# Huangtianyu-caas/MAGOT

Hardware: NVIDIA B200
Metric: spliced+translated Gbp/s (higher is better)
Workload: dtype u8

## Files before the change

magot_b200/csrc/mg_common.cuh:

```cuda
#pragma once
#include <cuda_runtime.h>
#include <stdint.h>
#include <stdio.h>
#include <atomic>
#include <string>
#include <vector>
#include "../../include/magot_b200.h"

#define MG_FRONT_PAD 64
#define MG_TAIL_WORDS 8
#define MG_CODE_EXC 15u

void mg_set_error(const char *fmt, ...);
extern std::atomic<int64_t> g_mg_launches;
#define MG_COUNT_LAUNCH() (++g_mg_launches)

#define MG_CUDA(call)                                                                             \
    do {                                                                                          \
        cudaError_t _e = (call);                                                                  \
        if (_e != cudaSuccess) {                                                                  \
            mg_set_error("%s failed at %s:%d: %s", #call, __FILE__, __LINE__, cudaGetErrorString(_e)); \
            return MG_ECUDA;                                                                      \
        }                                                                                         \
    } while (0)
// ... 35 lines not shown
    bool finalized = false;
    uint64_t generation = 0;
    uint8_t *d_stage = nullptr;
    int64_t stage_cap = 0;
    uint8_t *d_raw = nullptr;
    unsigned long long *d_strip_tmp = nullptr;
    int64_t raw_cap = 0;
    uint8_t *h_pin = nullptr;
    int64_t pin_cap = 0;
    uint8_t *d_aa4096 = nullptr;
    uint8_t *d_aa4096h = nullptr;
    uint32_t *d_stops = nullptr;
    int64_t stop_words = 0;
    bool stops_valid = false;
    uint32_t *d_stops_alt = nullptr;
    uint64_t stops_alt_key = 0;
    bool stops_alt_valid = false;
    mg_sixframe_state *six = nullptr;
    int64_t device_bytes = 0;
};

struct mg_plan {
    mg_genome *g = nullptr;
    int device = 0;
    int64_t n_rec = 0, n_seg = 0, n_piece = 0, n_lit = 0;
    int64_t *d_rec_seg_off = nullptr;
    int32_t *d_seg_contig = nullptr;
    int64_t *d_seg_start = nullptr, *d_seg_end = nullptr;
    int8_t *d_seg_strand = nullptr;
    int64_t *d_rec_lit_off = nullptr;
    int32_t *d_rec_pre = nullptr, *d_rec_suf = nullptr;
    int8_t *d_rec_phase = nullptr;
    uint8_t *d_lit = nullptr;
    int64_t *d_blk_r0 = nullptr;
    int64_t *d_piece_src = nullptr;
    int64_t *d_piece_off = nullptr;
    int64_t *d_prot_off = nullptr;
    int32_t *d_rec_aa = nullptr;
    int8_t *d_rec_skip = nullptr;
    int64_t *d_nuc_tile = nullptr;
    int64_t *d_prot_tile = nullptr;
    int64_t n_nuc_tile = 0, n_prot_tile = 0;
    int32_t *d_blk1k = nullptr;
    int64_t blk1k_cap = 0;
    bool blk1k_ready = false;
    int64_t max_seg_per_rec = 0;
    int64_t nuc_upper = 0;
    int64_t *d_tile_buf = nullptr;
    int64_t tile_cap = 0;
    cudaStream_t last_stream = 0;
    int64_t *d_scan_tmp = nullptr;
    int64_t scan_tmp_cap = 0;
    int64_t nuc_total = -1, prot_total = -1;
    int64_t *d_totals = nullptr;
    bool totals_known = false;
    int prot_flags = 0;
    bool prepared = false;
    uint64_t generation = 0;
    bool prot_ready = false;
    unsigned long long *rec_tmp = nullptr;
    int64_t rec_tmp_words = 0;
    int64_t *rec_tile = nullptr;
    uint32_t *d_order = nullptr;
    int64_t order_cap = 0;
    uint8_t *d_out = nullptr;
    int64_t out_cap = 0;
    uint8_t *d_aa8192 = nullptr;
    bool own_code = false;
    std::vector<void *> owned;
};

#define MG_KIND_FWD 0ull
#define MG_KIND_RC 1ull
#define MG_KIND_LIT 2ull
#define MG_KIND_SHIFT 62
#define MG_SRC_MASK ((1ull << MG_KIND_SHIFT) - 1ull)

#ifndef MG_NUC_TILE
#define MG_NUC_TILE 32768
#endif
#ifndef MG_PROT_TILE
#define MG_PROT_TILE 16384
#endif

void build_aa4096(uint8_t *t, const uint8_t *codon64);
int mg_plan_check_prepared(const mg_plan *p);
// ... 115 lines not shown
```

magot_b200/csrc/mg_plan.cu:

```cuda
#include <algorithm>
#include <cstdlib>
#include <cstring>
#include "mg_common.cuh"
#include "mg_gather.cuh"
#include "mg_lookback.cuh"


#define PLAN_ITEMS 4
#define PLAN_TILE (256 * PLAN_ITEMS)

__global__ void __launch_bounds__(256) k_plan_block_rec(int64_t n_block, int64_t n_rec, const int64_t *__restrict__ rec_seg_off,
                                                        int64_t *__restrict__ blk_r0) {
    const int64_t r = blockIdx.x * (int64_t)blockDim.x + threadIdx.x;
    if (r >= n_rec) return;
    const int64_t f0 = __ldg(rec_seg_off + r) + 2 * r, f1 = __ldg(rec_seg_off + r + 1) + 2 * (r + 1);
    for (int64_t b = (f0 + PLAN_TILE - 1) / PLAN_TILE; b * PLAN_TILE < f1 && b < n_block; b++) blk_r0[b] = r;
}

#ifndef PLAN_MINB
#define PLAN_MINB 8
#endif
__global__ void __launch_bounds__(256, PLAN_MINB) k_plan_pieces(int64_t n_piece, int64_t n_rec, const int64_t *__restrict__ rec_seg_off,
                                                     const int64_t *__restrict__ blk_r0,
                                                     const int32_t *__restrict__ seg_contig, const int64_t *__restrict__ seg_start,
                                                     const int64_t *__restrict__ seg_end, const int8_t *__restrict__ seg_strand,
                                                     const int64_t *__restrict__ rec_lit_off, const int32_t *__restrict__ rec_pre,
                                                     const int32_t *__restrict__ rec_suf, const int64_t *__restrict__ contig_len,
                                                     const int64_t *__restrict__ contig_base, int64_t n_contigs, int64_t two_T,
                                                     unsigned long long *tmp, int64_t *__restrict__ piece_off,
                                                     int64_t *__restrict__ piece_src, int64_t *__restrict__ total_out,
                                                     int64_t *__restrict__ tile_first, int64_t tile_cap,
                                                     int32_t *__restrict__ blk1k, int64_t blk1k_cap) {
    __shared__ int64_t s_F[PLAN_TILE / 2 + 2];
    __shared__ int64_t s_warp[8];
    __shared__ int64_t s_prefix;
    __shared__ unsigned int s_tile;
    const int64_t tile = mg_next_tile(tmp, &s_tile);
    const int64_t pb = tile * PLAN_TILE;
    const int64_t r0 = blk_r0[tile];
    for (int i = threadIdx.x; i < PLAN_TILE / 2 + 2; i += blockDim.x) {
        const int64_t r = r0 + i;
        s_F[i] = r <= n_rec ? __ldg(rec_seg_off + r) + 2 * r : INT64_MAX;
    }
    __syncthreads();
    int64_t len[PLAN_ITEMS];
    const int64_t p0 = pb + (int64_t)threadIdx.x * PLAN_ITEMS;
    int lo = 0;
#pragma unroll
    for (int it = 0; it < PLAN_ITEMS; it++) {
        const int64_t p = p0 + it;
        len[it] = 0;
        if (p < n_piece) {
            if (it == 0) {
                int hi = PLAN_TILE / 2 + 1;
                while (hi - lo > 1) {
                    const int mid = (lo + hi) >> 1;
                    if (s_F[mid] <= p) lo = mid; else hi = mid;
                }
            } else {
                while (s_F[lo + 1] <= p) lo++;
            }
            const int64_t r = r0 + lo;
            const int64_t s0 = s_F[lo] - 2 * r, s1 = s_F[lo + 1] - 2 * (r + 1);
            const int64_t local = p - (s0 + 2 * r);
            if (local == 0) {
                len[it] = rec_pre[r];
                piece_src[p] = rec_lit_off[r] | (int64_t)(MG_KIND_LIT << MG_KIND_SHIFT);
            } else if (local == s1 - s0 + 1) {
                len[it] = rec_suf[r];
                piece_src[p] = (rec_lit_off[r] + rec_pre[r]) | (int64_t)(MG_KIND_LIT << MG_KIND_SHIFT);
            } else {
                const int64_t e = s0 + local - 1;
                const int32_t c = seg_contig[e];
                int64_t src = MG_FRONT_PAD, n = 0;
                if (c >= 0 && c < n_contigs) {
                    const int64_t L = contig_len[c];
                    int64_t i = seg_start[e] - 1, j = seg_end[e];
                    if (i < 0) { i += L; if (i < 0) i = 0; } else if (i > L) i = L;
                    if (j < 0) { j += L; if (j < 0) j = 0; } else if (j > L) j = L;
                    n = j > i ? j - i : 0;
                    if (n > 0x7fffffff) n = 0x7fffffff;
                    src = contig_base[c] + i;
                }
                len[it] = n;
                piece_src[p] = seg_strand[e] ? two_T - src - n : src;
            }
        }
    }
    int64_t mine = 0;
#pragma unroll
    for (int it = 0; it < PLAN_ITEMS; it++) mine += len[it];
    int64_t total;
    const int64_t incl = mg_block_incl_scan(mine, s_warp, &total);
    const int64_t prefix = mg_lookback(tmp, tile, total, &s_prefix);
    int64_t run = prefix + incl - mine;
#pragma unroll
    for (int it = 0; it < PLAN_ITEMS; it++) {
        if (p0 + it < n_piece) {
            piece_off[p0 + it] = run;
            if (tile_first && len[it] > 0) {
                for (int64_t t = (run + MG_NUC_TILE - 1) / MG_NUC_TILE; t * MG_NUC_TILE < run + len[it] && t < tile_cap; t++)
                    tile_first[t] = p0 + it;
            }
            if (blk1k_cap > 0 && len[it] > 0) {
                for (int64_t t = (run + 1023) >> 10; (t << 10) < run + len[it] && t < blk1k_cap; t++) blk1k[t] = (int32_t)(p0 + it);
            }
        }
        run += len[it];
    }
    if (tile == gridDim.x - 1 && threadIdx.x == 0) {
        const int64_t all = prefix + total;
        piece_off[n_piece] = all;
        *total_out = all;
        if (tile_first) {
            const int64_t n_tile = min(tile_cap, (all + MG_NUC_TILE - 1) / MG_NUC_TILE);
            tile_first[n_tile] = n_piece > 0 ? n_piece - 1 : 0;
        }
        const int64_t n_blk = (all + 1023) >> 10;
        if (n_blk < blk1k_cap) blk1k[n_blk] = (int32_t)(n_piece > 0 ? n_piece - 1 : 0);
    }
}

__global__ void __launch_bounds__(256) k_plan_records(int64_t n_rec, const int64_t *__restrict__ rec_seg_off,
                                                      const int64_t *__restrict__ piece_off, const int64_t *__restrict__ piece_src,
                                                      const uint32_t *__restrict__ packed, const int8_t *__restrict__ rec_phase,
                                                      int flags, int32_t *__restrict__ rec_aa, int8_t *__restrict__ rec_skip,
                                                      unsigned long long *tmp, int64_t *__restrict__ prot_off,
                                                      int64_t *__restrict__ total_out, int64_t *__restrict__ tile_first,
                                                      int64_t tile_cap) {
    __shared__ int64_t s_warp[8];
    __shared__ int64_t s_prefix;
    __shared__ unsigned int s_tile;
    const int64_t tile = mg_next_tile(tmp, &s_tile);
    const int64_t r = tile * (int64_t)blockDim.x + threadIdx.x;
    int64_t plen = 0;
    if (r < n_rec) {
    const int64_t f0 = rec_seg_off[r] + 2 * r, f1 = rec_seg_off[r + 1] + 2 * (r + 1);
    const int64_t pay0 = piece_off[f0 + 1], pay1 = piece_off[f1 - 1];
    const int64_t pre = pay0 - piece_off[f0], suf = piece_off[f1] - pay1;
    int64_t L = pay1 - pay0;
    int skip = 0;
    if ((flags & MG_PROT_USE_PHASE) && rec_phase) { skip = rec_phase[r]; if (skip < 0 || skip > 2) skip = 0; }
    L -= skip;
    int64_t naa;
    if (L <= 2) {
        naa = -1;
    } else {
        naa = L / 3;
        if (flags & MG_PROT_TRIMX) {
            uint64_t acc[3];
            const int64_t S = pay0 + skip;
            int64_t j = f0 + 1;
            while (j + 1 < f1 - 1 && __ldg(piece_off + j + 1) <= S) j++;
            mg_gather_nib(packed, piece_off, piece_src, j, S, 3, acc);
            const uint32_t n3 = (uint32_t)acc[0] & 0xFFFu;
            if (n3 & 0x888u) { naa -= 1; skip += 3; }
        }
    }
    if (naa > 0x7fffffff) naa = 0x7fffffff;
    rec_aa[r] = (int32_t)naa;
    rec_skip[r] = (int8_t)skip;
    plen = pre + (naa > 0 ? naa : 0) + suf;
    }
    int64_t total;
    const int64_t incl = mg_block_incl_scan(plen, s_warp, &total);
    const int64_t prefix = mg_lookback(tmp, tile, total, &s_prefix);
    if (r < n_rec) {
        const int64_t off = prefix + incl - plen;
        prot_off[r] = off;
        if (tile_first && plen > 0) {
            for (int64_t t = (off + MG_PROT_TILE - 1) / MG_PROT_TILE; t * MG_PROT_TILE < off + plen && t < tile_cap; t++) tile_first[t] = r;
        }
    }
    if (tile == gridDim.x - 1 && threadIdx.x == blockDim.x - 1) {
        const int64_t all = prefix + total;
        prot_off[n_rec] = all;
        *total_out = all;
        if (tile_first) {
            const int64_t n_tile = min(tile_cap, (all + MG_PROT_TILE - 1) / MG_PROT_TILE);
            tile_first[n_tile] = n_rec > 0 ? n_rec - 1 : 0;
        }
    }
}


#define PR_THREADS 256
#ifndef PR_MAXSEG
#define PR_MAXSEG 256
#endif

struct pr_seg { int64_t src; int64_t n; };

__device__ __forceinline__ pr_seg pr_clamp(int64_t e, const int32_t *__restrict__ seg_contig, const int64_t *__restrict__ seg_start,
                                           const int64_t *__restrict__ seg_end, const int8_t *__restrict__ seg_strand,
                                           const int64_t *__restrict__ contig_len, const int64_t *__restrict__ contig_base,
                                           int64_t n_contigs, int64_t two_T) {
    const int32_t c = __ldg(seg_contig + e);
    int64_t src = MG_FRONT_PAD, n = 0;
    if (c >= 0 && c < n_contigs) {
        const int64_t L = __ldg(contig_len + c);
        int64_t i = __ldg(seg_start + e) - 1, j = __ldg(seg_end + e);
        if (i < 0) { i += L; if (i < 0) i = 0; } else if (i > L) i = L;
        if (j < 0) { j += L; if (j < 0) j = 0; } else if (j > L) j = L;
        n = j > i ? j - i : 0;
        if (n > 0x7fffffff) n = 0x7fffffff;
        src = __ldg(contig_base + c) + i;
    }
// ... 192 lines not shown
    MG_REQUIRE(n_seg == 0 || (seg_contig && seg_start && seg_end && seg_strand), "segment arrays are NULL");
    MG_REQUIRE(n_rec == 0 || (rec_lit_off && rec_pre_len && rec_suf_len), "record arrays are NULL");
    MG_REQUIRE(rec_seg_off[0] == 0 && rec_seg_off[n_rec] == n_seg, "rec_seg_off must start at 0 and end at n_seg");
    MG_REQUIRE(n_seg + 2 * n_rec < 0x7fffffff, "more than 2^31 pieces in one plan: split the table");
    MG_CUDA(cudaSetDevice(g->device));
    cudaStream_t st = (cudaStream_t)stream;
    mg_plan *p = new mg_plan();
    p->g = g;
    p->device = g->device;
    p->n_rec = n_rec;
    p->n_seg = n_seg;
    p->n_piece = n_seg + 2 * n_rec;
    p->n_lit = n_lit;
    p->last_stream = st;
    int rc = MG_OK;
#define TRY(x) do { rc = (x); if (rc) { mg_plan_destroy(p); return rc; } } while (0)
    TRY(upload(p, &p->d_rec_seg_off, rec_seg_off, n_rec + 1, st));
    TRY(upload(p, &p->d_seg_contig, seg_contig, n_seg, st));
    TRY(upload(p, &p->d_seg_start, seg_start, n_seg, st));
    TRY(upload(p, &p->d_seg_end, seg_end, n_seg, st));
    TRY(upload(p, &p->d_seg_strand, seg_strand, n_seg, st));
    TRY(upload(p, &p->d_rec_lit_off, rec_lit_off, n_rec, st));
    TRY(upload(p, &p->d_rec_pre, rec_pre_len, n_rec, st));
    TRY(upload(p, &p->d_rec_suf, rec_suf_len, n_rec, st));
    {
        uint8_t *d = nullptr;
        TRY(dalloc(p, &d, n_lit + 128, st));
        rc = cudaMemsetAsync(d, 0, n_lit + 128, st) == cudaSuccess ? MG_OK : MG_ECUDA;
        if (rc == MG_OK && n_lit > 0 && cudaMemcpyAsync(d + 64, lit, n_lit, cudaMemcpyHostToDevice, st) != cudaSuccess) rc = MG_ECUDA;
        if (rc) { mg_set_error("literal upload failed"); mg_plan_destroy(p); return rc; }
        p->d_lit = d + 64;
    }
    if (rec_phase) TRY(upload(p, &p->d_rec_phase, rec_phase, n_rec, st));
    TRY(dalloc(p, &p->d_blk_r0, (p->n_piece + PLAN_TILE - 1) / PLAN_TILE + 1, st));
    {
        int64_t up = 0;
        for (int64_t e = 0; e < n_seg; e++) {
            int64_t d = seg_end[e] - seg_start[e] + 1;
            const int32_t c = seg_contig[e];
            const int64_t L = (c >= 0 && c < g->n_contigs) ? g->h_contig_len[c] : 0;
            if (seg_start[e] > seg_end[e] || d > L) d = L;
            if (d > 0) up += d < 0x7fffffff ? d : 0x7fffffff;
        }
        for (int64_t r = 0; r < n_rec; r++) up += (int64_t)rec_pre_len[r] + rec_suf_len[r];
        p->nuc_upper = up;
        p->blk1k_cap = (up >> 10) + 3;
        TRY(dalloc(p, &p->d_blk1k, p->blk1k_cap, st));
    }
    TRY(dalloc(p, &p->d_piece_src, p->n_piece, st));
    TRY(dalloc(p, &p->d_piece_off, p->n_piece + 1, st));
    TRY(dalloc(p, &p->d_prot_off, n_rec + 1, st));
    TRY(dalloc(p, &p->d_rec_aa, n_rec, st));
    TRY(dalloc(p, &p->d_rec_skip, n_rec, st));
    p->scan_tmp_cap = (p->n_piece + PLAN_TILE - 1) / PLAN_TILE + 1 + 2 * ((n_rec + 127) / 128 + 1) + 2;
    for (int64_t r = 0; r < n_rec; r++) p->max_seg_per_rec = std::max(p->max_seg_per_rec, rec_seg_off[r + 1] - rec_seg_off[r]);
    TRY(dalloc(p, &p->d_scan_tmp, p->scan_tmp_cap, st));
#undef TRY
    if (n_rec > 0) {
        const int64_t n_block = (p->n_piece + PLAN_TILE - 1) / PLAN_TILE, n_rblock = (n_rec + 255) / 256;
        k_plan_block_rec<<<(unsigned)n_rblock, 256, 0, st>>>(n_block, n_rec, p->d_rec_seg_off, p->d_blk_r0);
        MG_COUNT_LAUNCH();
        if (cudaGetLastError() != cudaSuccess) { mg_set_error("k_plan_block_rec launch failed"); mg_plan_destroy(p); return MG_ECUDA; }
    }
    *out = p;
    return MG_OK;
}

extern "C" int mg_plan_destroy(mg_plan *p) {
    if (!p) return MG_OK;
    cudaSetDevice(p->device);
    for (void *d : p->owned) cudaFreeAsync(d, p->last_stream);
    if (p->d_out) cudaFreeAsync(p->d_out, p->last_stream);
    delete p;
    return MG_OK;
}

extern "C" int mg_plan_set_codon_table(mg_plan *p, const uint8_t *codon64) {
    MG_REQUIRE(p != nullptr, "plan handle is NULL");
    if (!codon64) { p->own_code = false; return MG_OK; }
    for (int c = 0; c < 64; c++) MG_REQUIRE(codon64[c] != 'X', "codon64 maps an A/C/G/T codon to 'X'");
    MG_CUDA(cudaSetDevice(p->device));
    uint8_t t[8192];
    build_aa4096(t, codon64);
    for (uint32_t c = 0; c < 4096; c++) t[4096 + mg_aa_slot(c)] = t[c];
    cudaStream_t st = p->last_stream;
    if (!p->d_aa8192) {
        int rc = dalloc(p, &p->d_aa8192, 8192, st);
        if (rc) return rc;
    }
    MG_CUDA(cudaMemcpyAsync(p->d_aa8192, t, 8192, cudaMemcpyHostToDevice, st));
    MG_CUDA(cudaStreamSynchronize(st));
    p->own_code = true;
    return MG_OK;
}

static int plan_alloc_tiles(mg_plan *p, int64_t cap_nuc, int64_t cap_prot, cudaStream_t st);
static int64_t plan_tile_need(int64_t cap_nuc, int64_t cap_prot) {
    return (cap_nuc + MG_NUC_TILE - 1) / MG_NUC_TILE + 1 + (cap_prot + MG_PROT_TILE - 1) / MG_PROT_TILE + 1;
}
static int64_t pr_tiles(const mg_plan *p) { return (p->n_rec + PR_RECS - 1) / PR_RECS; }

static int plan_launch_records(mg_plan *p, cudaStream_t st);
static int plan_launch_scans(mg_plan *p, int prot_flags, cudaStream_t st, bool scatter_tiles = false, int64_t cap_nuc = 0,
                             int64_t cap_prot = 0) {
    mg_genome *g = p->g;
    p->prot_flags = prot_flags;
    p->last_stream = st;
    p->prot_ready = false;
    const int64_t n_block = (p->n_piece + PLAN_TILE - 1) / PLAN_TILE, n_rblock = (p->n_rec + 255) / 256;
    unsigned long long *tmp_a = reinterpret_cast<unsigned long long *>(p->d_scan_tmp), *tmp_b = tmp_a + n_block + 1;
    p->d_totals = reinterpret_cast<int64_t *>(tmp_b + n_rblock + 1);
    const bool one_launch = p->n_rec > 0 && p->max_seg_per_rec <= PR_MAXSEG && mg_k1_mode() == 1;
    if (p->n_rec == 0) MG_CUDA(cudaMemsetAsync(p->d_scan_tmp, 0, p->scan_tmp_cap * sizeof(int64_t), st));
    else if (one_launch) MG_CUDA(cudaMemsetAsync(p->d_scan_tmp, 0, 2 * (pr_tiles(p) + 1) * sizeof(unsigned long long), st));
    else MG_CUDA(cudaMemsetAsync(tmp_a, 0, (n_block + 1) * sizeof(unsigned long long), st));
    int64_t *tf_nuc = nullptr, *tf_prot = nullptr;
    if (scatter_tiles) {
        int rc = plan_alloc_tiles(p, cap_nuc, cap_prot, st);
        if (rc) return rc;
        tf_nuc = p->d_nuc_tile;
        tf_prot = p->d_prot_tile;
    }
    if (p->n_rec == 0) { p->prot_ready = true; return MG_OK; }
    if (one_launch) {
        const int64_t n_tile = pr_tiles(p);
        unsigned long long *ta = reinterpret_cast<unsigned long long *>(p->d_scan_tmp), *tb = ta + n_tile + 1;
        p->d_totals = reinterpret_cast<int64_t *>(p->d_scan_tmp + p->scan_tmp_cap - 2);
        k_plan_rec<<<(unsigned)n_tile, PR_THREADS, 0, st>>>(
            p->n_rec, p->n_piece, p->d_rec_seg_off, p->d_seg_contig, p->d_seg_start, p->d_seg_end, p->d_seg_strand, p->d_rec_lit_off,
            p->d_rec_pre, p->d_rec_suf, p->d_rec_phase, prot_flags, g->d_contig_len, g->d_contig_base, g->n_contigs, 2 * g->total_bases,
            g->d_packed, ta, tb, p->d_piece_off, p->d_piece_src, p->d_prot_off, p->d_rec_aa, p->d_rec_skip, p->d_totals, tf_nuc,
            p->n_nuc_tile, tf_prot, p->n_prot_tile, p->d_blk1k, p->blk1k_cap);
        MG_LAUNCH_CHECK();
        p->prot_ready = true;
        p->blk1k_ready = true;
        return MG_OK;
    }
    const bool want_blk1k = mg_emit_mode() == 2;
    p->blk1k_ready = want_blk1k;
    k_plan_pieces<<<(unsigned)n_block, 256, 0, st>>>(
        p->n_piece, p->n_rec, p->d_rec_seg_off, p->d_blk_r0, p->d_seg_contig, p->d_seg_start, p->d_seg_end, p->d_seg_strand,
        p->d_rec_lit_off, p->d_rec_pre, p->d_rec_suf, g->d_contig_len, g->d_contig_base, g->n_contigs, 2 * g->total_bases,
        tmp_a, p->d_piece_off, p->d_piece_src, p->d_totals, tf_nuc, p->n_nuc_tile, p->d_blk1k, want_blk1k ? p->blk1k_cap : 0);
    MG_LAUNCH_CHECK();
    p->rec_tmp = tmp_b;
    p->rec_tmp_words = n_rblock + 1;
    p->rec_tile = tf_prot;
    if (prot_flags & MG_PROT_DEFER) return MG_OK;
    return plan_launch_records(p, st);
}

static int plan_launch_records(mg_plan *p, cudaStream_t st) {
    mg_genome *g = p->g;
    const int64_t n_rblock = (p->n_rec + 255) / 256;
    MG_CUDA(cudaMemsetAsync(p->rec_tmp, 0, p->rec_tmp_words * sizeof(unsigned long long), st));
    k_plan_records<<<(unsigned)n_rblock, 256, 0, st>>>(
        p->n_rec, p->d_rec_seg_off, p->d_piece_off, p->d_piece_src, g->d_packed, p->d_rec_phase, p->prot_flags,
        p->d_rec_aa, p->d_rec_skip, p->rec_tmp, p->d_prot_off, p->d_totals + 1, p->rec_tile, p->n_prot_tile);
    MG_LAUNCH_CHECK();
    p->prot_ready = true;
    return MG_OK;
}

int mg_plan_check_prepared(const mg_plan *p) {
    if (!p->prepared) { mg_set_error("mg_plan_prepare has not been called"); return MG_ESTATE; }
    if (p->generation != p->g->generation) {
        mg_set_error("the genome changed (pack, finalize or mask) since the plan was prepared: prepare it again");
        return MG_ESTATE;
    }
    return MG_OK;
}

extern "C" int mg_plan_prepare_prot_async(mg_plan *p, void *stream) {
    MG_REQUIRE(p != nullptr, "plan handle is NULL");
    if (!p->prepared) { mg_set_error("mg_plan_prepare_async has not been called"); return MG_ESTATE; }
    if (const int rc0 = mg_plan_check_prepared(p)) return rc0;
    if (p->prot_ready || p->n_rec == 0) return MG_OK;
    MG_CUDA(cudaSetDevice(p->device));
    p->last_stream = (cudaStream_t)stream;
    return plan_launch_records(p, (cudaStream_t)stream);
}

static int plan_alloc_tiles(mg_plan *p, int64_t cap_nuc, int64_t cap_prot, cudaStream_t st) {
    p->n_nuc_tile = (cap_nuc + MG_NUC_TILE - 1) / MG_NUC_TILE;
    p->n_prot_tile = (cap_prot + MG_PROT_TILE - 1) / MG_PROT_TILE;
    const int64_t tile_need = plan_tile_need(cap_nuc, cap_prot);
    if (tile_need > p->tile_cap) {
        void *d = nullptr;
        MG_CUDA(cudaMallocAsync(&d, tile_need * sizeof(int64_t), st));
        p->owned.push_back(d);
        p->d_tile_buf = (int64_t *)d;
        p->tile_cap = tile_need;
    }
    p->d_nuc_tile = p->d_tile_buf;
    p->d_prot_tile = p->d_tile_buf + p->n_nuc_tile + 1;
    return MG_OK;
}

static int plan_launch_tiles(mg_plan *p, int64_t cap_nuc, int64_t cap_prot, cudaStream_t st) {
    int rc = plan_alloc_tiles(p, cap_nuc, cap_prot, st);
    if (rc) return rc;
    if (p->n_rec > 0 && p->n_nuc_tile + p->n_prot_tile > 0) {
        k_plan_tiles<<<(unsigned)((p->n_nuc_tile + p->n_prot_tile + 2 + 255) / 256), 256, 0, st>>>(
            p->d_totals, p->d_piece_off, p->n_piece, MG_NUC_TILE, p->n_nuc_tile, p->d_nuc_tile, p->d_prot_off, p->n_rec, MG_PROT_TILE,
            p->n_prot_tile, p->d_prot_tile);
        MG_LAUNCH_CHECK();
    }
    return MG_OK;
}

static int plan_read_totals(mg_plan *p, cudaStream_t st, int64_t totals[2]) {
    totals[0] = totals[1] = 0;
// ... 9 lines not shown
    MG_CUDA(cudaSetDevice(p->device));
    cudaStream_t st = (cudaStream_t)stream;
    p->prepared = false;
    int rc = plan_launch_scans(p, prot_flags & ~MG_PROT_DEFER, st);
    if (rc) return rc;
    int64_t totals[2];
    rc = plan_read_totals(p, st, totals);
    if (rc) return rc;
    p->nuc_total = totals[0];
    p->prot_total = totals[1];
    p->totals_known = true;
    rc = plan_launch_tiles(p, p->nuc_total, p->prot_total, st);
    if (rc) return rc;
    p->prepared = true;
    p->generation = p->g->generation;
    if (nuc_total) *nuc_total = p->nuc_total;
    if (prot_total) *prot_total = p->prot_total;
    return MG_OK;
}

extern "C" int mg_plan_prepare_async(mg_plan *p, int prot_flags, int64_t nuc_capacity, int64_t prot_capacity, void *stream) {
    MG_REQUIRE(p != nullptr, "plan handle is NULL");
    MG_REQUIRE(nuc_capacity >= 0 && prot_capacity >= 0, "capacities must be >= 0");
    MG_CUDA(cudaSetDevice(p->device));
    if (plan_tile_need(nuc_capacity, prot_capacity) > p->tile_cap) {
        const int rc0 = mg_refuse_growth_in_capture((cudaStream_t)stream, "mg_plan_prepare_async (first prepare, or larger capacities)");
        if (rc0) return rc0;
    }
    p->prepared = false;
    int rc = plan_launch_scans(p, prot_flags, (cudaStream_t)stream, true, nuc_capacity, prot_capacity);
    if (rc) return rc;
    p->nuc_total = nuc_capacity;
    p->prot_total = prot_capacity;
    p->totals_known = false;
    p->prepared = true;
    p->generation = p->g->generation;
    return MG_OK;
}

extern "C" int mg_plan_totals(mg_plan *p, int64_t *nuc_total, int64_t *prot_total, void *stream) {
    MG_REQUIRE(p != nullptr, "plan handle is NULL");
    if (const int rc0 = mg_plan_check_prepared(p)) return rc0;
    MG_CUDA(cudaSetDevice(p->device));
    if (!p->totals_known) {
        int64_t totals[2];
        int rc = plan_read_totals(p, (cudaStream_t)stream, totals);
        if (rc) return rc;
        if (!p->prot_ready) totals[1] = 0;
        if (totals[0] > p->nuc_total || totals[1] > p->prot_total) {
            mg_set_error("text sizes (%lld nucleotide, %lld protein bytes) exceed the capacities given to mg_plan_prepare_async "
                         "(%lld, %lld): the emitted texts are truncated", (long long)totals[0], (long long)totals[1],
                         (long long)p->nuc_total, (long long)p->prot_total);
            return MG_EINVAL;
        }
        p->nuc_total = totals[0];
        p->prot_total = totals[1];
        p->totals_known = true;
    }
    if (nuc_total) *nuc_total = p->nuc_total;
    if (prot_total) *prot_total = p->prot_total;
    return MG_OK;
}

extern "C" int mg_plan_lengths(mg_plan *p, int64_t *nuc_len, int64_t *aa_len, void *stream) {
    MG_REQUIRE(p != nullptr, "plan handle is NULL");
    if (const int rc0 = mg_plan_check_prepared(p)) return rc0;
// ... 16 lines not shown
```

Measured before the change: 1938.

## Precompute per-piece descriptors to replace binary search in plan pieces kernel

Replaces the per-tile record index and the shared-memory binary search in k_plan_pieces with a precomputed int32 descriptor per piece: either a segment index, or an encoded record prefix/suffix literal. The pieces kernel then reads the descriptors with vector loads and issues segment and literal loads in batches to raise memory-level parallelism, keeping lengths in shared memory. Tile-first and blk1k writes are skipped when a thread's range does not cross a tile boundary. The record kernel gains a fast path that reads the first codon directly when it lies within the first piece. In exchange it adds an n_piece-sized descriptor buffer and limits indices to 32 bits.

Result: faster. 1976, median of 6 (+2.0%).

```diff
diff --git a/magot_b200/csrc/mg_common.cuh b/magot_b200/csrc/mg_common.cuh
--- a/magot_b200/csrc/mg_common.cuh
+++ b/magot_b200/csrc/mg_common.cuh
@@ -91,7 +91,7 @@
     int32_t *d_rec_pre = nullptr, *d_rec_suf = nullptr;
     int8_t *d_rec_phase = nullptr;
     uint8_t *d_lit = nullptr;
-    int64_t *d_blk_r0 = nullptr;
+    int32_t *d_piece_desc = nullptr;
     int64_t *d_piece_src = nullptr;
     int64_t *d_piece_off = nullptr;
     int64_t *d_prot_off = nullptr;
diff --git a/magot_b200/csrc/mg_plan.cu b/magot_b200/csrc/mg_plan.cu
--- a/magot_b200/csrc/mg_plan.cu
+++ b/magot_b200/csrc/mg_plan.cu
@@ -6,22 +6,28 @@
 #include "mg_lookback.cuh"
 
 
+#ifndef PLAN_ITEMS
 #define PLAN_ITEMS 4
+#endif
 #define PLAN_TILE (256 * PLAN_ITEMS)
-
-__global__ void __launch_bounds__(256) k_plan_block_rec(int64_t n_block, int64_t n_rec, const int64_t *__restrict__ rec_seg_off,
-                                                        int64_t *__restrict__ blk_r0) {
-    const int64_t r = blockIdx.x * (int64_t)blockDim.x + threadIdx.x;
+#ifndef PLAN_ILP
+#define PLAN_ILP 2
+#endif
+
+__global__ void __launch_bounds__(256) k_plan_desc(int64_t n_rec, const int64_t *__restrict__ rec_seg_off, int32_t *__restrict__ desc) {
+    const int64_t r = (blockIdx.x * (int64_t)blockDim.x + threadIdx.x) >> 5;
+    const int lane = threadIdx.x & 31;
     if (r >= n_rec) return;
-    const int64_t f0 = __ldg(rec_seg_off + r) + 2 * r, f1 = __ldg(rec_seg_off + r + 1) + 2 * (r + 1);
-    for (int64_t b = (f0 + PLAN_TILE - 1) / PLAN_TILE; b * PLAN_TILE < f1 && b < n_block; b++) blk_r0[b] = r;
+    const int64_t s0 = __ldg(rec_seg_off + r), s1 = __ldg(rec_seg_off + r + 1), f0 = s0 + 2 * r;
+    if (lane == 0) desc[f0] = ~(int32_t)(2 * r);
+    if (lane == 1) desc[s1 + 2 * r + 1] = ~(int32_t)(2 * r + 1);
+    for (int64_t k = lane; k < s1 - s0; k += 32) desc[f0 + 1 + k] = (int32_t)(s0 + k);
 }
 
 #ifndef PLAN_MINB
 #define PLAN_MINB 8
 #endif
-__global__ void __launch_bounds__(256, PLAN_MINB) k_plan_pieces(int64_t n_piece, int64_t n_rec, const int64_t *__restrict__ rec_seg_off,
-                                                     const int64_t *__restrict__ blk_r0,
+__global__ void __launch_bounds__(256, PLAN_MINB) k_plan_pieces(int64_t n_piece, const int32_t *__restrict__ desc,
                                                      const int32_t *__restrict__ seg_contig, const int64_t *__restrict__ seg_start,
                                                      const int64_t *__restrict__ seg_end, const int8_t *__restrict__ seg_strand,
                                                      const int64_t *__restrict__ rec_lit_off, const int32_t *__restrict__ rec_pre,
@@ -31,82 +37,90 @@
                                                      int64_t *__restrict__ piece_src, int64_t *__restrict__ total_out,
                                                      int64_t *__restrict__ tile_first, int64_t tile_cap,
                                                      int32_t *__restrict__ blk1k, int64_t blk1k_cap) {
-    __shared__ int64_t s_F[PLAN_TILE / 2 + 2];
+    __shared__ int32_t s_len[256 * (PLAN_ITEMS + 1)];
     __shared__ int64_t s_warp[8];
     __shared__ int64_t s_prefix;
     __shared__ unsigned int s_tile;
     const int64_t tile = mg_next_tile(tmp, &s_tile);
-    const int64_t pb = tile * PLAN_TILE;
-    const int64_t r0 = blk_r0[tile];
-    for (int i = threadIdx.x; i < PLAN_TILE / 2 + 2; i += blockDim.x) {
-        const int64_t r = r0 + i;
-        s_F[i] = r <= n_rec ? __ldg(rec_seg_off + r) + 2 * r : INT64_MAX;
-    }
-    __syncthreads();
-    int64_t len[PLAN_ITEMS];
-    const int64_t p0 = pb + (int64_t)threadIdx.x * PLAN_ITEMS;
-    int lo = 0;
-#pragma unroll
-    for (int it = 0; it < PLAN_ITEMS; it++) {
-        const int64_t p = p0 + it;
-        len[it] = 0;
-        if (p < n_piece) {
-            if (it == 0) {
-                int hi = PLAN_TILE / 2 + 1;
-                while (hi - lo > 1) {
-                    const int mid = (lo + hi) >> 1;
-                    if (s_F[mid] <= p) lo = mid; else hi = mid;
-                }
-            } else {
-                while (s_F[lo + 1] <= p) lo++;
-            }
-            const int64_t r = r0 + lo;
-            const int64_t s0 = s_F[lo] - 2 * r, s1 = s_F[lo + 1] - 2 * (r + 1);
-            const int64_t local = p - (s0 + 2 * r);
-            if (local == 0) {
-                len[it] = rec_pre[r];
-                piece_src[p] = rec_lit_off[r] | (int64_t)(MG_KIND_LIT << MG_KIND_SHIFT);
-            } else if (local == s1 - s0 + 1) {
-                len[it] = rec_suf[r];
-                piece_src[p] = (rec_lit_off[r] + rec_pre[r]) | (int64_t)(MG_KIND_LIT << MG_KIND_SHIFT);
-            } else {
-                const int64_t e = s0 + local - 1;
-                const int32_t c = seg_contig[e];
-                int64_t src = MG_FRONT_PAD, n = 0;
-                if (c >= 0 && c < n_contigs) {
-                    const int64_t L = contig_len[c];
-                    int64_t i = seg_start[e] - 1, j = seg_end[e];
-                    if (i < 0) { i += L; if (i < 0) i = 0; } else if (i > L) i = L;
-                    if (j < 0) { j += L; if (j < 0) j = 0; } else if (j > L) j = L;
-                    n = j > i ? j - i : 0;
-                    if (n > 0x7fffffff) n = 0x7fffffff;
-                    src = contig_base[c] + i;
-                }
-                len[it] = n;
-                piece_src[p] = seg_strand[e] ? two_T - src - n : src;
-            }
-        }
-    }
+    const int64_t p0 = tile * PLAN_TILE + (int64_t)threadIdx.x * PLAN_ITEMS;
+    const int nv = (int)max((int64_t)0, min((int64_t)PLAN_ITEMS, n_piece - p0));
+    int32_t *len = s_len + threadIdx.x * (PLAN_ITEMS + 1);
     int64_t mine = 0;
 #pragma unroll
-    for (int it = 0; it < PLAN_ITEMS; it++) mine += len[it];
+    for (int q = 0; q < PLAN_ITEMS; q += 4) {
+        int32_t d[4];
+        if (q + 4 <= nv) {
+            const int4 v = __ldg(reinterpret_cast<const int4 *>(desc + p0 + q));
+            d[0] = v.x; d[1] = v.y; d[2] = v.z; d[3] = v.w;
+        } else {
+#pragma unroll
+            for (int k = 0; k < 4; k++) d[k] = q + k < nv ? __ldg(desc + p0 + q + k) : 0;
+        }
+#pragma unroll
+        for (int h = 0; h < 4; h += PLAN_ILP) {
+            int32_t c[PLAN_ILP], X[PLAN_ILP];
+            int64_t A[PLAN_ILP], B[PLAN_ILP];
+#pragma unroll
+            for (int k = 0; k < PLAN_ILP; k++) {
+                const int it = q + h + k;
+                const int32_t di = d[h + k];
+                const bool seg = it < nv && di >= 0, lp = it < nv && di < 0;
+                const int32_t e = seg ? di : 0, r = lp ? (~di) >> 1 : 0;
+                c[k] = seg ? __ldg(seg_contig + e) : -1;
+                A[k] = seg ? __ldg(seg_start + e) - 1 : (lp ? __ldg(rec_lit_off + r) : 0);
+                B[k] = seg ? __ldg(seg_end + e) : (lp ? (int64_t)__ldg(rec_pre + r) : 0);
+                X[k] = seg ? (int32_t)__ldg(seg_strand + e) : ((lp && (~di & 1)) ? __ldg(rec_suf + r) : 0);
+            }
+#pragma unroll
+            for (int k = 0; k < PLAN_ILP; k++) {
+                const int it = q + h + k;
+                const int32_t di = d[h + k];
+                const bool ok = c[k] >= 0 && c[k] < n_contigs;
+                const int64_t L = ok ? __ldg(contig_len + c[k]) : 0, base = ok ? __ldg(contig_base + c[k]) : 0;
+                int64_t a = A[k], b = B[k];
+                if (a < 0) { a += L; if (a < 0) a = 0; } else if (a > L) a = L;
+                if (b < 0) { b += L; if (b < 0) b = 0; } else if (b > L) b = L;
+                int64_t m = ok && b > a ? b - a : 0;
+                if (m > 0x7fffffff) m = 0x7fffffff;
+                const int64_t s = ok ? base + a : MG_FRONT_PAD;
+                const bool is_suf = (~di) & 1;
+                const int64_t src = di >= 0 ? (X[k] ? two_T - s - m : s)
+                                            : (A[k] + (is_suf ? B[k] : 0)) | (int64_t)(MG_KIND_LIT << MG_KIND_SHIFT);
+                const int32_t n = it < nv ? (di >= 0 ? (int32_t)m : (int32_t)(is_suf ? X[k] : B[k])) : 0;
+                if (it < nv) piece_src[p0 + it] = src;
+                mine += n;
+                len[it] = n;
+            }
+        }
+    }
     int64_t total;
     const int64_t incl = mg_block_incl_scan(mine, s_warp, &total);
     const int64_t prefix = mg_lookback(tmp, tile, total, &s_prefix);
-    int64_t run = prefix + incl - mine;
+    const int64_t start = prefix + incl - mine;
+    int64_t run = start;
 #pragma unroll
     for (int it = 0; it < PLAN_ITEMS; it++) {
-        if (p0 + it < n_piece) {
-            piece_off[p0 + it] = run;
-            if (tile_first && len[it] > 0) {
-                for (int64_t t = (run + MG_NUC_TILE - 1) / MG_NUC_TILE; t * MG_NUC_TILE < run + len[it] && t < tile_cap; t++)
-                    tile_first[t] = p0 + it;
-            }
-            if (blk1k_cap > 0 && len[it] > 0) {
-                for (int64_t t = (run + 1023) >> 10; (t << 10) < run + len[it] && t < blk1k_cap; t++) blk1k[t] = (int32_t)(p0 + it);
-            }
-        }
+        if (it < nv) piece_off[p0 + it] = run;
         run += len[it];
+    }
+    bool neg = start < 0;
+#pragma unroll
+    for (int it = 0; it < PLAN_ITEMS; it++) neg |= len[it] < 0;
+    if (tile_first && (neg || ((start + MG_NUC_TILE - 1) / MG_NUC_TILE) * MG_NUC_TILE < run)) {
+        int64_t o = start;
+        for (int it = 0; it < nv; it++) {
+            if (len[it] > 0)
+                for (int64_t t = (o + MG_NUC_TILE - 1) / MG_NUC_TILE; t * MG_NUC_TILE < o + len[it] && t < tile_cap; t++) tile_first[t] = p0 + it;
+            o += len[it];
+        }
+    }
+    if (blk1k_cap > 0) {
+        int64_t o = start;
+        for (int it = 0; it < nv; it++) {
+            if (len[it] > 0)
+                for (int64_t t = (o + 1023) >> 10; (t << 10) < o + len[it] && t < blk1k_cap; t++) blk1k[t] = (int32_t)(p0 + it);
+            o += len[it];
+        }
     }
     if (tile == gridDim.x - 1 && threadIdx.x == 0) {
         const int64_t all = prefix + total;
@@ -135,9 +149,11 @@
     const int64_t r = tile * (int64_t)blockDim.x + threadIdx.x;
     int64_t plen = 0;
     if (r < n_rec) {
-    const int64_t f0 = rec_seg_off[r] + 2 * r, f1 = rec_seg_off[r + 1] + 2 * (r + 1);
-    const int64_t pay0 = piece_off[f0 + 1], pay1 = piece_off[f1 - 1];
-    const int64_t pre = pay0 - piece_off[f0], suf = piece_off[f1] - pay1;
+    const int64_t f0 = __ldg(rec_seg_off + r) + 2 * r, f1 = __ldg(rec_seg_off + r + 1) + 2 * (r + 1);
+    const int64_t pay0 = __ldg(piece_off + f0 + 1), pay1 = __ldg(piece_off + f1 - 1);
+    const int64_t pre = pay0 - __ldg(piece_off + f0), suf = __ldg(piece_off + f1) - pay1;
+    const int64_t end1 = __ldg(piece_off + f0 + 2);
+    const uint64_t src1 = (uint64_t)__ldg(piece_src + f0 + 1);
     int64_t L = pay1 - pay0;
     int skip = 0;
     if ((flags & MG_PROT_USE_PHASE) && rec_phase) { skip = rec_phase[r]; if (skip < 0 || skip > 2) skip = 0; }
@@ -148,12 +164,17 @@
     } else {
         naa = L / 3;
         if (flags & MG_PROT_TRIMX) {
-            uint64_t acc[3];
-            const int64_t S = pay0 + skip;
-            int64_t j = f0 + 1;
-            while (j + 1 < f1 - 1 && __ldg(piece_off + j + 1) <= S) j++;
-            mg_gather_nib(packed, piece_off, piece_src, j, S, 3, acc);
-            const uint32_t n3 = (uint32_t)acc[0] & 0xFFFu;
+            uint32_t n3;
+            if (end1 - pay0 >= skip + 3) {
+                n3 = (uint32_t)mg_ld_nib16(packed, (int64_t)(src1 & MG_SRC_MASK) + skip) & 0xFFFu;
+            } else {
+                uint64_t acc[3];
+                const int64_t S = pay0 + skip;
+                int64_t j = f0 + 1;
+                while (j + 1 < f1 - 1 && __ldg(piece_off + j + 1) <= S) j++;
+                mg_gather_nib(packed, piece_off, piece_src, j, S, 3, acc);
+                n3 = (uint32_t)acc[0] & 0xFFFu;
+            }
             if (n3 & 0x888u) { naa -= 1; skip += 3; }
         }
     }
@@ -431,7 +452,7 @@
         p->d_lit = d + 64;
     }
     if (rec_phase) TRY(upload(p, &p->d_rec_phase, rec_phase, n_rec, st));
-    TRY(dalloc(p, &p->d_blk_r0, (p->n_piece + PLAN_TILE - 1) / PLAN_TILE + 1, st));
+    TRY(dalloc(p, &p->d_piece_desc, p->n_piece, st));
     {
         int64_t up = 0;
         for (int64_t e = 0; e < n_seg; e++) {
@@ -456,10 +477,9 @@
     TRY(dalloc(p, &p->d_scan_tmp, p->scan_tmp_cap, st));
 #undef TRY
     if (n_rec > 0) {
-        const int64_t n_block = (p->n_piece + PLAN_TILE - 1) / PLAN_TILE, n_rblock = (n_rec + 255) / 256;
-        k_plan_block_rec<<<(unsigned)n_rblock, 256, 0, st>>>(n_block, n_rec, p->d_rec_seg_off, p->d_blk_r0);
+        k_plan_desc<<<(unsigned)((n_rec + 7) / 8), 256, 0, st>>>(n_rec, p->d_rec_seg_off, p->d_piece_desc);
         MG_COUNT_LAUNCH();
-        if (cudaGetLastError() != cudaSuccess) { mg_set_error("k_plan_block_rec launch failed"); mg_plan_destroy(p); return MG_ECUDA; }
+        if (cudaGetLastError() != cudaSuccess) { mg_set_error("k_plan_desc launch failed"); mg_plan_destroy(p); return MG_ECUDA; }
     }
     *out = p;
     return MG_OK;
@@ -538,7 +558,7 @@
     const bool want_blk1k = mg_emit_mode() == 2;
     p->blk1k_ready = want_blk1k;
     k_plan_pieces<<<(unsigned)n_block, 256, 0, st>>>(
-        p->n_piece, p->n_rec, p->d_rec_seg_off, p->d_blk_r0, p->d_seg_contig, p->d_seg_start, p->d_seg_end, p->d_seg_strand,
+        p->n_piece, p->d_piece_desc, p->d_seg_contig, p->d_seg_start, p->d_seg_end, p->d_seg_strand,
         p->d_rec_lit_off, p->d_rec_pre, p->d_rec_suf, g->d_contig_len, g->d_contig_base, g->n_contigs, 2 * g->total_bases,
         tmp_a, p->d_piece_off, p->d_piece_src, p->d_totals, tf_nuc, p->n_nuc_tile, p->d_blk1k, want_blk1k ? p->blk1k_cap : 0);
     MG_LAUNCH_CHECK();
```

## Restructure plan kernels: bitmap record heads, coalesced piece work, multi-record threads

Applied to the files above, without the earlier changes.

Rewrites k_plan_pieces so each tile marks record boundaries in a shared bitmap and ranks them with popcount instead of a per-thread binary search. Per-piece segment work is spread across threads in a coalesced stride, and offsets are staged in shared memory so the scatter pass is also coalesced. The tile is doubled to 8 items per thread with lower minimum blocks per SM. k_plan_records now handles two records per thread and reads the first codon straight from packed memory when it lies inside one piece; a protein-total reset fix is bundled in. This adds shared-memory pressure and more complex indexing, with a risk of off-by-one errors at tile edges.

Result: faster. 1950 before, 2036 after, median of 6 (+4.4%).

```diff
diff --git a/magot_b200/csrc/mg_common.cuh b/magot_b200/csrc/mg_common.cuh
--- a/magot_b200/csrc/mg_common.cuh
+++ b/magot_b200/csrc/mg_common.cuh
@@ -111,6 +111,7 @@
     int64_t *d_scan_tmp = nullptr;
     int64_t scan_tmp_cap = 0;
     int64_t nuc_total = -1, prot_total = -1;
+    int64_t prot_cap = 0;
     int64_t *d_totals = nullptr;
     bool totals_known = false;
     int prot_flags = 0;
diff --git a/magot_b200/csrc/mg_plan.cu b/magot_b200/csrc/mg_plan.cu
--- a/magot_b200/csrc/mg_plan.cu
+++ b/magot_b200/csrc/mg_plan.cu
@@ -6,8 +6,12 @@
 #include "mg_lookback.cuh"
 
 
-#define PLAN_ITEMS 4
-#define PLAN_TILE (256 * PLAN_ITEMS)
+#define PLAN_THREADS 256
+#ifndef PLAN_ITEMS
+#define PLAN_ITEMS 8
+#endif
+#define PLAN_TILE (PLAN_THREADS * PLAN_ITEMS)
+#define PLAN_WORDS (PLAN_TILE / 32)
 
 __global__ void __launch_bounds__(256) k_plan_block_rec(int64_t n_block, int64_t n_rec, const int64_t *__restrict__ rec_seg_off,
                                                         int64_t *__restrict__ blk_r0) {
@@ -17,10 +21,18 @@
     for (int64_t b = (f0 + PLAN_TILE - 1) / PLAN_TILE; b * PLAN_TILE < f1 && b < n_block; b++) blk_r0[b] = r;
 }
 
+__device__ __forceinline__ void plan_scatter_nuc(int64_t off, int64_t len, int64_t p, int64_t *__restrict__ tile_first,
+                                                 int64_t tile_cap, int32_t *__restrict__ blk1k, int64_t blk1k_cap) {
+    if (len <= 0) return;
+    if (tile_first)
+        for (int64_t t = (off + MG_NUC_TILE - 1) / MG_NUC_TILE; t * MG_NUC_TILE < off + len && t < tile_cap; t++) tile_first[t] = p;
+    for (int64_t t = (off + 1023) >> 10; (t << 10) < off + len && t < blk1k_cap; t++) blk1k[t] = (int32_t)p;
+}
+
 #ifndef PLAN_MINB
-#define PLAN_MINB 8
+#define PLAN_MINB 6
 #endif
-__global__ void __launch_bounds__(256, PLAN_MINB) k_plan_pieces(int64_t n_piece, int64_t n_rec, const int64_t *__restrict__ rec_seg_off,
+__global__ void __launch_bounds__(PLAN_THREADS, PLAN_MINB) k_plan_pieces(int64_t n_piece, int64_t n_rec, const int64_t *__restrict__ rec_seg_off,
                                                      const int64_t *__restrict__ blk_r0,
                                                      const int32_t *__restrict__ seg_contig, const int64_t *__restrict__ seg_start,
                                                      const int64_t *__restrict__ seg_end, const int8_t *__restrict__ seg_strand,
@@ -31,82 +43,117 @@
                                                      int64_t *__restrict__ piece_src, int64_t *__restrict__ total_out,
                                                      int64_t *__restrict__ tile_first, int64_t tile_cap,
                                                      int32_t *__restrict__ blk1k, int64_t blk1k_cap) {
-    __shared__ int64_t s_F[PLAN_TILE / 2 + 2];
+    __shared__ __align__(16) int64_t s_buf[PLAN_TILE];
+    uint32_t *s_len = reinterpret_cast<uint32_t *>(s_buf);
+    __shared__ uint32_t s_head[PLAN_WORDS + 1];
+    __shared__ uint32_t s_cnt[PLAN_WORDS];
     __shared__ int64_t s_warp[8];
     __shared__ int64_t s_prefix;
     __shared__ unsigned int s_tile;
+    for (int i = threadIdx.x; i <= PLAN_WORDS; i += PLAN_THREADS) s_head[i] = 0;
     const int64_t tile = mg_next_tile(tmp, &s_tile);
     const int64_t pb = tile * PLAN_TILE;
+    const int nt = (int)min((int64_t)PLAN_TILE, n_piece - pb);
+    const int64_t pe = pb + nt;
     const int64_t r0 = blk_r0[tile];
-    for (int i = threadIdx.x; i < PLAN_TILE / 2 + 2; i += blockDim.x) {
-        const int64_t r = r0 + i;
-        s_F[i] = r <= n_rec ? __ldg(rec_seg_off + r) + 2 * r : INT64_MAX;
+
+    for (int64_t r = r0 + threadIdx.x;; r += PLAN_THREADS) {
+        bool more = false;
+        if (r < n_rec) {
+            const int64_t f0 = __ldg(rec_seg_off + r) + 2 * r;
+            if (f0 < pe) {
+                const int64_t f1 = __ldg(rec_seg_off + r + 1) + 2 * (r + 1);
+                const int64_t lit = __ldg(rec_lit_off + r);
+                const int32_t pre = __ldg(rec_pre + r), suf = __ldg(rec_suf + r);
+                if (f0 >= pb) {
+                    s_len[f0 - pb] = (uint32_t)pre;
+                    piece_src[f0] = lit | (int64_t)(MG_KIND_LIT << MG_KIND_SHIFT);
+                    if (f0 == pb) atomicOr(&s_head[0], 1u);
+                }
+                if (f1 - 1 < pe) {
+                    s_len[f1 - 1 - pb] = (uint32_t)suf;
+                    piece_src[f1 - 1] = (lit + pre) | (int64_t)(MG_KIND_LIT << MG_KIND_SHIFT);
+                }
+                if (f1 - pb <= PLAN_TILE) atomicOr(&s_head[(f1 - pb) >> 5], 1u << ((f1 - pb) & 31));
+                more = f1 < pe;
+            }
+        }
+        if (!__syncthreads_and(more)) break;
+    }
+    if (threadIdx.x < 32) {
+        uint32_t c[PLAN_WORDS / 32], sum = 0;
+#pragma unroll
+        for (int k = 0; k < PLAN_WORDS / 32; k++) { c[k] = __popc(s_head[threadIdx.x * (PLAN_WORDS / 32) + k]); sum += c[k]; }
+        uint32_t incl = sum;
+#pragma unroll
+        for (int d = 1; d < 32; d <<= 1) {
+            const uint32_t t = __shfl_up_sync(0xffffffffu, incl, d);
+            if ((int)threadIdx.x >= d) incl += t;
+        }
+        uint32_t run = incl - sum;
+#pragma unroll
+        for (int k = 0; k < PLAN_WORDS / 32; k++) { s_cnt[threadIdx.x * (PLAN_WORDS / 32) + k] = run; run += c[k]; }
     }
     __syncthreads();
-    int64_t len[PLAN_ITEMS];
-    const int64_t p0 = pb + (int64_t)threadIdx.x * PLAN_ITEMS;
-    int lo = 0;
-#pragma unroll
+
+    const int lane = threadIdx.x & 31;
+    const uint32_t upto = 0xffffffffu >> (31 - lane);
+    const int64_t rb = r0 - (int64_t)(s_head[0] & 1u);
+#pragma unroll 4
     for (int it = 0; it < PLAN_ITEMS; it++) {
-        const int64_t p = p0 + it;
-        len[it] = 0;
-        if (p < n_piece) {
-            if (it == 0) {
-                int hi = PLAN_TILE / 2 + 1;
-                while (hi - lo > 1) {
-                    const int mid = (lo + hi) >> 1;
-                    if (s_F[mid] <= p) lo = mid; else hi = mid;
-                }
-            } else {
-                while (s_F[lo + 1] <= p) lo++;
-            }
-            const int64_t r = r0 + lo;
-            const int64_t s0 = s_F[lo] - 2 * r, s1 = s_F[lo + 1] - 2 * (r + 1);
-            const int64_t local = p - (s0 + 2 * r);
-            if (local == 0) {
-                len[it] = rec_pre[r];
-                piece_src[p] = rec_lit_off[r] | (int64_t)(MG_KIND_LIT << MG_KIND_SHIFT);
-            } else if (local == s1 - s0 + 1) {
-                len[it] = rec_suf[r];
-                piece_src[p] = (rec_lit_off[r] + rec_pre[r]) | (int64_t)(MG_KIND_LIT << MG_KIND_SHIFT);
-            } else {
-                const int64_t e = s0 + local - 1;
-                const int32_t c = seg_contig[e];
-                int64_t src = MG_FRONT_PAD, n = 0;
-                if (c >= 0 && c < n_contigs) {
-                    const int64_t L = contig_len[c];
-                    int64_t i = seg_start[e] - 1, j = seg_end[e];
-                    if (i < 0) { i += L; if (i < 0) i = 0; } else if (i > L) i = L;
-                    if (j < 0) { j += L; if (j < 0) j = 0; } else if (j > L) j = L;
-                    n = j > i ? j - i : 0;
-                    if (n > 0x7fffffff) n = 0x7fffffff;
-                    src = contig_base[c] + i;
-                }
-                len[it] = n;
-                piece_src[p] = seg_strand[e] ? two_T - src - n : src;
-            }
-        }
-    }
+        const int j = it * PLAN_THREADS + threadIdx.x, w = j >> 5;
+        if (j >= nt) { s_len[j] = 0; continue; }
+        const uint32_t h = s_head[w];
+        const uint32_t lit = h | (h >> 1) | (s_head[w + 1] << 31);
+        if ((lit >> lane) & 1u) continue;
+        const int64_t p = pb + j;
+        const int64_t e = p - 2 * (rb + s_cnt[w] + __popc(h & upto)) - 1;
+        const int32_t c = __ldg(seg_contig + e);
+        const int64_t s = __ldg(seg_start + e), en = __ldg(seg_end + e);
+        const int8_t minus = __ldg(seg_strand + e);
+        int64_t src = MG_FRONT_PAD, n = 0;
+        if (c >= 0 && c < n_contigs) {
+            const int64_t L = __ldg(contig_len + c);
+            int64_t i = s - 1, k = en;
+            if (i < 0) { i += L; if (i < 0) i = 0; } else if (i > L) i = L;
+            if (k < 0) { k += L; if (k < 0) k = 0; } else if (k > L) k = L;
+            n = k > i ? k - i : 0;
+            if (n > 0x7fffffff) n = 0x7fffffff;
+            src = __ldg(contig_base + c) + i;
+        }
+        s_len[j] = (uint32_t)n;
+        piece_src[p] = minus ? two_T - src - n : src;
+    }
+    __syncthreads();
+
+    uint32_t len[PLAN_ITEMS];
     int64_t mine = 0;
 #pragma unroll
-    for (int it = 0; it < PLAN_ITEMS; it++) mine += len[it];
+    for (int q = 0; q < PLAN_ITEMS / 4; q++) {
+        const uint4 u = reinterpret_cast<const uint4 *>(s_len + threadIdx.x * PLAN_ITEMS)[q];
+        len[4 * q] = u.x; len[4 * q + 1] = u.y; len[4 * q + 2] = u.z; len[4 * q + 3] = u.w;
+        mine += (int64_t)u.x + (int64_t)u.y + (int64_t)u.z + (int64_t)u.w;
+    }
     int64_t total;
     const int64_t incl = mg_block_incl_scan(mine, s_warp, &total);
+    int64_t run = incl - mine;
+#pragma unroll
+    for (int i = 0; i < PLAN_ITEMS; i++) {
+        s_buf[threadIdx.x * PLAN_ITEMS + ((i + threadIdx.x) & (PLAN_ITEMS - 1))] = run;
+        run += len[i];
+    }
     const int64_t prefix = mg_lookback(tmp, tile, total, &s_prefix);
-    int64_t run = prefix + incl - mine;
-#pragma unroll
+
+#pragma unroll 4
     for (int it = 0; it < PLAN_ITEMS; it++) {
-        if (p0 + it < n_piece) {
-            piece_off[p0 + it] = run;
-            if (tile_first && len[it] > 0) {
-                for (int64_t t = (run + MG_NUC_TILE - 1) / MG_NUC_TILE; t * MG_NUC_TILE < run + len[it] && t < tile_cap; t++)
-                    tile_first[t] = p0 + it;
-            }
-            if (blk1k_cap > 0 && len[it] > 0) {
-                for (int64_t t = (run + 1023) >> 10; (t << 10) < run + len[it] && t < blk1k_cap; t++) blk1k[t] = (int32_t)(p0 + it);
-            }
-        }
-        run += len[it];
+        const int j = it * PLAN_THREADS + threadIdx.x;
+        if (j >= nt) break;
+        const int t0 = j / PLAN_ITEMS, t1 = (j + 1) / PLAN_ITEMS;
+        const int64_t o0 = s_buf[t0 * PLAN_ITEMS + ((j + t0) & (PLAN_ITEMS - 1))];
+        const int64_t o1 = j + 1 < nt ? s_buf[t1 * PLAN_ITEMS + ((j + 1 + t1) & (PLAN_ITEMS - 1))] : total;
+        const int64_t off = prefix + o0;
+        piece_off[pb + j] = off;
+        plan_scatter_nuc(off, o1 - o0, pb + j, tile_first, tile_cap, blk1k, blk1k_cap);
     }
     if (tile == gridDim.x - 1 && threadIdx.x == 0) {
         const int64_t all = prefix + total;
@@ -121,7 +168,12 @@
     }
 }
 
-__global__ void __launch_bounds__(256) k_plan_records(int64_t n_rec, const int64_t *__restrict__ rec_seg_off,
+#define REC_THREADS 256
+#ifndef REC_ITEMS
+#define REC_ITEMS 2
+#endif
+#define REC_TILE (REC_THREADS * REC_ITEMS)
+__global__ void __launch_bounds__(REC_THREADS) k_plan_records(int64_t n_rec, const int64_t *__restrict__ rec_seg_off,
                                                       const int64_t *__restrict__ piece_off, const int64_t *__restrict__ piece_src,
                                                       const uint32_t *__restrict__ packed, const int8_t *__restrict__ rec_phase,
                                                       int flags, int32_t *__restrict__ rec_aa, int8_t *__restrict__ rec_skip,
@@ -132,47 +184,68 @@
     __shared__ int64_t s_prefix;
     __shared__ unsigned int s_tile;
     const int64_t tile = mg_next_tile(tmp, &s_tile);
-    const int64_t r = tile * (int64_t)blockDim.x + threadIdx.x;
-    int64_t plen = 0;
-    if (r < n_rec) {
-    const int64_t f0 = rec_seg_off[r] + 2 * r, f1 = rec_seg_off[r + 1] + 2 * (r + 1);
-    const int64_t pay0 = piece_off[f0 + 1], pay1 = piece_off[f1 - 1];
-    const int64_t pre = pay0 - piece_off[f0], suf = piece_off[f1] - pay1;
-    int64_t L = pay1 - pay0;
-    int skip = 0;
-    if ((flags & MG_PROT_USE_PHASE) && rec_phase) { skip = rec_phase[r]; if (skip < 0 || skip > 2) skip = 0; }
-    L -= skip;
-    int64_t naa;
-    if (L <= 2) {
-        naa = -1;
-    } else {
-        naa = L / 3;
-        if (flags & MG_PROT_TRIMX) {
-            uint64_t acc[3];
-            const int64_t S = pay0 + skip;
-            int64_t j = f0 + 1;
-            while (j + 1 < f1 - 1 && __ldg(piece_off + j + 1) <= S) j++;
-            mg_gather_nib(packed, piece_off, piece_src, j, S, 3, acc);
-            const uint32_t n3 = (uint32_t)acc[0] & 0xFFFu;
-            if (n3 & 0x888u) { naa -= 1; skip += 3; }
-        }
-    }
-    if (naa > 0x7fffffff) naa = 0x7fffffff;
-    rec_aa[r] = (int32_t)naa;
-    rec_skip[r] = (int8_t)skip;
-    plen = pre + (naa > 0 ? naa : 0) + suf;
+    const int64_t r0 = tile * REC_TILE + (int64_t)threadIdx.x * REC_ITEMS;
+    const bool phase = (flags & MG_PROT_USE_PHASE) && rec_phase;
+    int64_t so[REC_ITEMS + 1];
+    int ph[REC_ITEMS];
+#pragma unroll
+    for (int k = 0; k <= REC_ITEMS; k++) so[k] = r0 + k <= n_rec ? __ldg(rec_seg_off + r0 + k) : 0;
+#pragma unroll
+    for (int k = 0; k < REC_ITEMS; k++) ph[k] = phase && r0 + k < n_rec ? rec_phase[r0 + k] : 0;
+    int64_t plen[REC_ITEMS], mine = 0;
+#pragma unroll
+    for (int k = 0; k < REC_ITEMS; k++) {
+        const int64_t r = r0 + k;
+        plen[k] = 0;
+        if (r >= n_rec) continue;
+        const int64_t f0 = so[k] + 2 * r, f1 = so[k + 1] + 2 * (r + 1);
+        const int64_t o_pre = __ldg(piece_off + f0), pay0 = __ldg(piece_off + f0 + 1), o_2 = __ldg(piece_off + f0 + 2);
+        const int64_t pay1 = __ldg(piece_off + f1 - 1), o_end = __ldg(piece_off + f1);
+        const int64_t src1 = __ldg(piece_src + f0 + 1) & (int64_t)MG_SRC_MASK;
+        int skip = ph[k];
+        if (skip < 0 || skip > 2) skip = 0;
+        const int64_t L = pay1 - pay0 - skip;
+        int64_t naa;
+        if (L <= 2) {
+            naa = -1;
+        } else {
+            naa = L / 3;
+            if (flags & MG_PROT_TRIMX) {
+                const int64_t S = pay0 + skip;
+                uint32_t n3;
+                if (S + 3 <= o_2) {
+                    n3 = (uint32_t)mg_ld_nib16(packed, src1 + skip);
+                } else {
+                    uint64_t acc[3];
+                    int64_t j = f0 + 1;
+                    while (j + 1 < f1 - 1 && __ldg(piece_off + j + 1) <= S) j++;
+                    mg_gather_nib(packed, piece_off, piece_src, j, S, 3, acc);
+                    n3 = (uint32_t)acc[0];
+                }
+                if (n3 & 0x888u) { naa -= 1; skip += 3; }
+            }
+        }
+        if (naa > 0x7fffffff) naa = 0x7fffffff;
+        rec_aa[r] = (int32_t)naa;
+        rec_skip[r] = (int8_t)skip;
+        plen[k] = (pay0 - o_pre) + (naa > 0 ? naa : 0) + (o_end - pay1);
+        mine += plen[k];
     }
     int64_t total;
-    const int64_t incl = mg_block_incl_scan(plen, s_warp, &total);
+    const int64_t incl = mg_block_incl_scan(mine, s_warp, &total);
     const int64_t prefix = mg_lookback(tmp, tile, total, &s_prefix);
-    if (r < n_rec) {
-        const int64_t off = prefix + incl - plen;
+    int64_t off = prefix + incl - mine;
+#pragma unroll
+    for (int k = 0; k < REC_ITEMS; k++) {
+        const int64_t r = r0 + k;
+        if (r >= n_rec) break;
         prot_off[r] = off;
-        if (tile_first && plen > 0) {
-            for (int64_t t = (off + MG_PROT_TILE - 1) / MG_PROT_TILE; t * MG_PROT_TILE < off + plen && t < tile_cap; t++) tile_first[t] = r;
-        }
-    }
-    if (tile == gridDim.x - 1 && threadIdx.x == blockDim.x - 1) {
+        if (tile_first && plen[k] > 0) {
+            for (int64_t t = (off + MG_PROT_TILE - 1) / MG_PROT_TILE; t * MG_PROT_TILE < off + plen[k] && t < tile_cap; t++) tile_first[t] = r;
+        }
+        off += plen[k];
+    }
+    if (tile == gridDim.x - 1 && threadIdx.x == 0) {
         const int64_t all = prefix + total;
         prot_off[n_rec] = all;
         *total_out = all;
@@ -506,7 +579,7 @@
     p->prot_flags = prot_flags;
     p->last_stream = st;
     p->prot_ready = false;
-    const int64_t n_block = (p->n_piece + PLAN_TILE - 1) / PLAN_TILE, n_rblock = (p->n_rec + 255) / 256;
+    const int64_t n_block = (p->n_piece + PLAN_TILE - 1) / PLAN_TILE, n_rblock = (p->n_rec + REC_TILE - 1) / REC_TILE;
     unsigned long long *tmp_a = reinterpret_cast<unsigned long long *>(p->d_scan_tmp), *tmp_b = tmp_a + n_block + 1;
     p->d_totals = reinterpret_cast<int64_t *>(tmp_b + n_rblock + 1);
     const bool one_launch = p->n_rec > 0 && p->max_seg_per_rec <= PR_MAXSEG && mg_k1_mode() == 1;
@@ -537,7 +610,7 @@
     }
     const bool want_blk1k = mg_emit_mode() == 2;
     p->blk1k_ready = want_blk1k;
-    k_plan_pieces<<<(unsigned)n_block, 256, 0, st>>>(
+    k_plan_pieces<<<(unsigned)n_block, PLAN_THREADS, 0, st>>>(
         p->n_piece, p->n_rec, p->d_rec_seg_off, p->d_blk_r0, p->d_seg_contig, p->d_seg_start, p->d_seg_end, p->d_seg_strand,
         p->d_rec_lit_off, p->d_rec_pre, p->d_rec_suf, g->d_contig_len, g->d_contig_base, g->n_contigs, 2 * g->total_bases,
         tmp_a, p->d_piece_off, p->d_piece_src, p->d_totals, tf_nuc, p->n_nuc_tile, p->d_blk1k, want_blk1k ? p->blk1k_cap : 0);
@@ -551,9 +624,9 @@
 
 static int plan_launch_records(mg_plan *p, cudaStream_t st) {
     mg_genome *g = p->g;
-    const int64_t n_rblock = (p->n_rec + 255) / 256;
+    const int64_t n_rblock = (p->n_rec + REC_TILE - 1) / REC_TILE;
     MG_CUDA(cudaMemsetAsync(p->rec_tmp, 0, p->rec_tmp_words * sizeof(unsigned long long), st));
-    k_plan_records<<<(unsigned)n_rblock, 256, 0, st>>>(
+    k_plan_records<<<(unsigned)n_rblock, REC_THREADS, 0, st>>>(
         p->n_rec, p->d_rec_seg_off, p->d_piece_off, p->d_piece_src, g->d_packed, p->d_rec_phase, p->prot_flags,
         p->d_rec_aa, p->d_rec_skip, p->rec_tmp, p->d_prot_off, p->d_totals + 1, p->rec_tile, p->n_prot_tile);
     MG_LAUNCH_CHECK();
@@ -577,6 +650,10 @@
     if (p->prot_ready || p->n_rec == 0) return MG_OK;
     MG_CUDA(cudaSetDevice(p->device));
     p->last_stream = (cudaStream_t)stream;
+    if (p->totals_known) {
+        p->prot_total = p->prot_cap;
+        p->totals_known = false;
+    }
     return plan_launch_records(p, (cudaStream_t)stream);
 }
 
@@ -652,6 +729,7 @@
     if (rc) return rc;
     p->nuc_total = nuc_capacity;
     p->prot_total = prot_capacity;
+    p->prot_cap = prot_capacity;
     p->totals_known = false;
     p->prepared = true;
     p->generation = p->g->generation;
```
